# brain-research/l2hmc

Measured on AMD Instinct MI355X. Metric: chain_leapfrog_steps_per_sec, higher is better.
Workload: dtype f32

## Files before the change

### include/l2hmc.h

```cpp
#ifndef L2HMC_H_
#define L2HMC_H_

#include <stdint.h>

#ifdef __cplusplus
extern "C" {
#endif

#define L2HMC_ABI_VERSION 6

enum {
  L2HMC_OK = 0,
  L2HMC_ERR_ARG = -1,
  L2HMC_ERR_UNSUPPORTED = -2,
  L2HMC_ERR_HIP = -3
};

enum {
  L2HMC_ENERGY_GAUSS_DIAG = 1,
  L2HMC_ENERGY_GAUSS_DENSE = 2,
  L2HMC_ENERGY_GMM = 3,
  L2HMC_ENERGY_ROUGHWELL = 4,
  L2HMC_ENERGY_FUNNEL = 5,
  L2HMC_ENERGY_LOGISTIC = 7
// ... 182 lines not shown
  int64_t n_chains;
  int32_t d, H, T;
  const float* x;
  const float* v;
  const uint8_t* direction;
  int32_t direction_all;
  float scale;
  float inv_n;
  float* Lx;
  float* p;
  float* v1;
  float* grad;
  float* workspace;
  int32_t variant;
} L2hmcTrainArgs;

int64_t l2hmc_train_workspace_floats(int64_t n_chains, int32_t d, int32_t H, int32_t T);
int64_t l2hmc_train_grad_floats(int32_t d, int32_t H);
int64_t l2hmc_train_fused_lds_bytes(int32_t energy_kind, int32_t n_comp, int32_t d, int32_t H, int32_t T);
int64_t l2hmc_train_logistic_lds_bytes(int32_t n_data, int32_t d, int32_t H, int32_t T);
int l2hmc_train_propose_grad(const L2hmcTrainArgs* args, void* stream);

typedef struct L2hmcTrainStep {
  const float* x_head;
  int64_t n_head;
  const float* u;
  float* x_next;
  float* terms;
  double* loss;
  float* theta;
// ... 90 lines not shown
```

### l2hmc_amd/_ffi.py

```python
import ctypes as C
import os

_HERE = os.path.dirname(os.path.abspath(__file__))
LIB_PATH = os.path.abspath(os.environ["L2HMC_LIB"]) if os.environ.get("L2HMC_LIB") else os.path.join(_HERE, "csrc", "libl2hmc_hip.so")

ENERGY_GAUSS_DIAG, ENERGY_GAUSS_DENSE, ENERGY_GMM, ENERGY_ROUGHWELL, ENERGY_FUNNEL = 1, 2, 3, 4, 5
ENERGY_LOGISTIC = 7

_fp = C.c_void_p

NET_FIELDS = ("W1", "b1", "W2", "b2", "W3", "b3", "W4", "b4",
              "Ws", "bs", "Wt", "bt", "Wq", "bq", "lam_s", "lam_q")


class L2hmcNet(C.Structure):
    _fields_ = [(k, _fp) for k in NET_FIELDS]


class L2hmcEnergy(C.Structure):
    _fields_ = [("kind", C.c_int32), ("n_comp", C.c_int32), ("mu", _fp), ("prec", _fp),
                ("logc", _fp), ("eta", C.c_float), ("easy", C.c_int32),
                ("temperature", C.c_float), ("anneal_beta", C.c_float),
                ("den", C.c_float), ("reserved_", C.c_int32)]

# ... 99 lines not shown
    "l2hmc_pack_gaussian": (C.c_int, [_fp, C.c_int32, _fp, _fp]),
    "l2hmc_packed_logistic_floats": (C.c_int64, [C.c_int32, C.c_int32]),
    "l2hmc_pack_logistic": (C.c_int, [_fp, _fp, C.c_int32, C.c_int32, _fp, _fp]),
    "l2hmc_trajectory": (C.c_int, [C.POINTER(L2hmcTrajectoryArgs), _fp]),
    "l2hmc_trajectory_ladder": (C.c_int, [C.POINTER(L2hmcTrajectoryArgs), C.POINTER(L2hmcLadderArgs), _fp]),
    "l2hmc_energy": (C.c_int, [C.POINTER(L2hmcEnergy), _fp, C.c_int64, C.c_int32, _fp, _fp, _fp]),
    "l2hmc_p_accept": (C.c_int, [C.POINTER(L2hmcEnergy), _fp, _fp, _fp, _fp, _fp, C.c_int64,
                                 C.c_int32, _fp, _fp]),
    "l2hmc_mh_select": (C.c_int, [_fp, _fp, _fp, _fp, C.c_int64, C.c_int32, _fp, _fp]),
    "l2hmc_loss_terms": (C.c_int, [_fp, C.c_int64, C.c_float, C.c_double, _fp, _fp]),
    "l2hmc_split_workspace_floats": (C.c_int64, [C.c_int64, C.c_int32, C.c_int32, C.c_int32,
                                                 C.POINTER(L2hmcMlp3), C.POINTER(L2hmcMlp3)]),
    "l2hmc_trajectory_split": (C.c_int, [C.POINTER(L2hmcSplitArgs), _fp]),
    "l2hmc_vae_energy": (C.c_int, [C.POINTER(L2hmcMlp3), _fp, _fp, C.c_int64, C.c_int32, _fp, _fp, _fp, C.c_float, _fp]),
    "l2hmc_p_accept_energies": (C.c_int, [_fp, _fp, _fp, _fp, _fp, C.c_int64, C.c_int32, _fp, _fp]),
    "l2hmc_train_workspace_floats": (C.c_int64, [C.c_int64, C.c_int32, C.c_int32, C.c_int32]),
    "l2hmc_train_grad_floats": (C.c_int64, [C.c_int32, C.c_int32]),
    "l2hmc_train_fused_lds_bytes": (C.c_int64, [C.c_int32, C.c_int32, C.c_int32, C.c_int32, C.c_int32]),
    "l2hmc_train_logistic_lds_bytes": (C.c_int64, [C.c_int32, C.c_int32, C.c_int32, C.c_int32]),
    "l2hmc_train_propose_grad": (C.c_int, [C.POINTER(L2hmcTrainArgs), _fp]),
    "l2hmc_train_step": (C.c_int, [C.POINTER(L2hmcTrainArgs), C.POINTER(L2hmcTrainStep), _fp]),
    "l2hmc_adam_step_terms": (C.c_int, [_fp, _fp, _fp, _fp, C.c_int64, C.c_float, C.c_float, C.c_float, C.c_float,
                                        C.c_int64, C.c_int32, _fp, C.c_float, _fp, _fp]),
    "l2hmc_train_split_grad_floats": (C.c_int64, [C.c_int32, C.c_int32, C.POINTER(L2hmcMlp3)]),
    "l2hmc_train_split_workspace_floats": (C.c_int64, [C.c_int64, C.c_int32, C.c_int32, C.c_int32,
                                                       C.POINTER(L2hmcMlp3), C.POINTER(L2hmcMlp3)]),
    "l2hmc_train_split_grad": (C.c_int, [C.POINTER(L2hmcTrainSplitArgs), _fp]),
    "l2hmc_adam_step": (C.c_int, [_fp, _fp, _fp, _fp, C.c_int64, C.c_float, C.c_float, C.c_float, C.c_float,
                                  C.c_int64, C.c_int32, _fp]),
    "l2hmc_ais_begin_step": (C.c_int, [_fp, _fp, _fp, C.c_float, C.c_float, _fp, _fp, C.c_int64, C.c_int32, _fp]),
# ... 68 lines not shown
```

### l2hmc_amd/csrc/l2hmc_abi.hip

```cpp
#include <cstdlib>
#include "traj_tile.hpp"
#include "traj_lane.hpp"

namespace l2hmc {

thread_local char g_err[512] = "";
thread_local char g_kernel[96] = "";
void note_kernel(const char* fmt, long long a, long long b, long long c, long long d) { snprintf(g_kernel, sizeof(g_kernel), fmt, a, b, c, d); }

int fail(int code, const char* fmt, const char* a, long long b, long long c) {
  snprintf(g_err, sizeof(g_err), fmt, a, b, c);
  return code;
}

__global__ void pack_net_kernel(L2hmcNet net, int d, int H, int KH, int NT, float* out) {
  const int idx = blockIdx.x * blockDim.x + threadIdx.x;
  const int ngf = net_groups(NT) * 256;
  if (idx >= net_floats(NT)) return;
  float val = 0.f;
  if (idx < ngf) {
    const int g = idx >> 8, lane = (idx >> 2) & 63, r = idx & 3;
    const int i = lane & 15, q = lane >> 4;
    const int ui = ((i & 3) < KH) ? (i >> 2) * KH + (i & 3) : -1;
    const int uk = (r < KH) ? q * KH + r : -1;
// ... 319 lines not shown
  const int NT = k.NT, DP = 16 * NT, NTp = NW * DT;
  long long o = 0;
  k.o_fw = (int)o;
  o += 2LL * fast_fw_net(NTp, f16);
  k.o_fc = (int)o;
  o += 2LL * fast_fc_net(NTp);
  k.o_rec = (int)o;
  o += 2LL * fast_rec_dir(NTp, k.T);
  k.o_P = (int)o;
  if (NW > 1) o += 2LL * NW * 256;
  k.xb_stride = DP + 4;
  k.o_XB = (int)o;
  if (NW > 1 && (k.ekind == L2HMC_ENERGY_GAUSS_DENSE || k.ekind == L2HMC_ENERGY_GMM)) o += 16LL * k.xb_stride;
  k.o_red = (int)o;
  o += (long long)NW * 16 * 8;
  const int nc = k.ekind == L2HMC_ENERGY_GMM ? k.ncomp : 1;
  k.o_mu = (int)o;
  o += (long long)nc * DP;
  k.o_prec = (int)o;
  if (k.ekind == L2HMC_ENERGY_GAUSS_DIAG) o += DP;
  if (k.ekind == L2HMC_ENERGY_GAUSS_DENSE || k.ekind == L2HMC_ENERGY_GMM) o += (long long)nc * gauss_floats(NT);
  k.o_logc = (int)o;
  o += round4(nc);
  return o * 4;
}

long long plan_lds_tile(KArgs& k, int DT) {
  long long o = 0;
  k.o_fw = (int)o;
  o += 2LL * tile_fw_net(DT);
// ... 297 lines not shown
const char* l2hmc_last_error(void) { return g_err; }

int64_t l2hmc_struct_bytes(int32_t which) {
  switch (which) {
    case L2HMC_STRUCT_NET: return sizeof(L2hmcNet);
    case L2HMC_STRUCT_ENERGY: return sizeof(L2hmcEnergy);
    case L2HMC_STRUCT_TRAJECTORY_ARGS: return sizeof(L2hmcTrajectoryArgs);
    case L2HMC_STRUCT_MLP3: return sizeof(L2hmcMlp3);
    case L2HMC_STRUCT_SPLIT_ARGS: return sizeof(L2hmcSplitArgs);
    case L2HMC_STRUCT_TRAIN_ARGS: return sizeof(L2hmcTrainArgs);
    case L2HMC_STRUCT_TRAIN_SPLIT_ARGS: return sizeof(L2hmcTrainSplitArgs);
    case L2HMC_STRUCT_TRAIN_STEP: return sizeof(L2hmcTrainStep);
    case L2HMC_STRUCT_LADDER_ARGS: return sizeof(L2hmcLadderArgs);
  }
  return fail(L2HMC_ERR_ARG, "l2hmc_struct_bytes: unknown struct id%s");
}

int64_t l2hmc_packed_nets_floats(int32_t d, int32_t H) {
  if (d < 1 || H < 1) return fail(L2HMC_ERR_ARG, "d and H must be >= 1%s");
  if (H > 15) return fail(L2HMC_ERR_UNSUPPORTED, "fused nets support H <= 15 (got %s%lld)", "", H);
  if (d > 512) return fail(L2HMC_ERR_UNSUPPORTED, "fused nets support d <= 512 (got %s%lld)", "", d);
  return 2LL * net_floats(tiles_of(d)) + 2LL * lane_layout(d, H).total + 2LL * net_f16_floats(tiles_of(d));
}

int l2hmc_pack_nets(const L2hmcNet* xnet, const L2hmcNet* vnet, int32_t d, int32_t H,
                    float* packed, void* stream) {
  const int64_t n = l2hmc_packed_nets_floats(d, H);
  if (n < 0) return (int)n;
  if (!xnet || !vnet || !packed) return fail(L2HMC_ERR_ARG, "l2hmc_pack_nets: NULL argument%s");
  const L2hmcNet* nets[2] = {xnet, vnet};
// ... 357 lines not shown
```

### l2hmc_amd/csrc/l2hmc_kernels.hpp

```cpp
#pragma once
#include <hip/hip_runtime.h>
#include <stdint.h>
#include <stdio.h>
#include <string.h>
#include <type_traits>

#include "../../include/l2hmc.h"

namespace l2hmc {

typedef float f4 __attribute__((ext_vector_type(4)));

#define MFMA16(a, b, c) __builtin_amdgcn_mfma_f32_16x16x4f32((a), (b), (c), 0, 0, 0)

__host__ __device__ constexpr bool weights_in_global(int DT) { return DT >= 4; }

int fail(int code, const char* fmt, const char* a = "", long long b = 0, long long c = 0);
inline float roughwell_den(const L2hmcEnergy* e) {
  if (e->den > 0.f) return e->den;
  return e->easy ? e->eta : (float)((double)e->eta * (double)e->eta);
}
void note_kernel(const char* fmt, long long a = 0, long long b = 0, long long c = 0, long long d = 0);
inline bool adam_args_ok(float lr, float beta1, float beta2, float epsilon, int64_t step) {
  return step >= 1 && lr >= 0.f && (beta1 >= 0.f && beta1 < 1.f) && (beta2 >= 0.f && beta2 < 1.f) && epsilon > 0.f;
// ... 50 lines not shown
  long long chain_off;
  int ekind, ncomp, easy;
  const float *mu, *prec, *logc;
  float eta, temperature;
  float den;
  float beta;
  const float *x1, *v1, *logjac_in;
  float *U_out, *grad_out;
  int o_mask, o_trig, o_tb, o_P, o_XB, o_red, o_mu, o_prec, o_logc, xb_stride;
  int o_state;
  const float* ais_beta;
  const float* ais_v0;
  float ais_dbeta, ais_refresh;
  float *ais_w, *ais_alpha;
  int o_fw, o_fc, o_rec;
  unsigned long long* dbg;
};

struct LadArgs {
  int K, M;
  int o_lad;
  float temp[16];
  unsigned long long round0;
  signed char *rung, *trip, *rung_hist;
  const float* u;
  float* cold;
  long long *acc, *att, *trips;
};

#ifdef L2HMC_PHASE_TIMING
// ... 109 lines not shown
  return (fabsf(p) <= 3.402823466e38f) ? p : 0.f;
}

struct U4 { unsigned x, y, z, w; };
__host__ __device__ inline U4 philox4x32_10(U4 c, unsigned k0, unsigned k1) {
#pragma unroll
  for (int i = 0; i < 10; ++i) {
    const unsigned long long p0 = 0xD2511F53ull * c.x, p1 = 0xCD9E8D57ull * c.z;
    const U4 n = {(unsigned)(p1 >> 32) ^ c.y ^ k0, (unsigned)p1, (unsigned)(p0 >> 32) ^ c.w ^ k1, (unsigned)p0};
    c = n;
    k0 += 0x9E3779B9u;
    k1 += 0xBB67AE85u;
  }
  return c;
}
__device__ __forceinline__ f4 philox_normal4(unsigned long long seed, long long gchain, unsigned blk,
                                             unsigned long long prop) {
  const U4 r = philox4x32_10(U4{(unsigned)gchain, blk, (unsigned)prop, (unsigned)(prop >> 32) << 1},
                             (unsigned)seed, (unsigned)(seed >> 32));
  const float k = 5.9604644775390625e-08f;
  const float u1 = ((r.x >> 8) + 1) * k, u2 = (r.y >> 8) * k, u3 = ((r.z >> 8) + 1) * k, u4 = (r.w >> 8) * k;
#ifdef L2HMC_LIBM_NORMALS
  const float ra = sqrtf(-2.f * logf(u1)), rb = sqrtf(-2.f * logf(u3));
  float sa, ca, sb, cb;
  sincosf(6.283185307179586f * u2, &sa, &ca);
  sincosf(6.283185307179586f * u4, &sb, &cb);
#else
  const float m2ln2 = -1.3862943611198906f;
  const float ra = __builtin_amdgcn_sqrtf(m2ln2 * __builtin_amdgcn_logf(u1)), rb = __builtin_amdgcn_sqrtf(m2ln2 * __builtin_amdgcn_logf(u3));
  const float sa = __builtin_amdgcn_sinf(u2), ca = __builtin_amdgcn_cosf(u2), sb = __builtin_amdgcn_sinf(u4), cb = __builtin_amdgcn_cosf(u4);
#endif
  return f4{ra * ca, ra * sa, rb * cb, rb * sb};
}
__device__ __forceinline__ void philox_dir_u(unsigned long long seed, long long gchain,
                                             unsigned long long prop, bool& fwd, float& u) {
  const U4 r = philox4x32_10(U4{(unsigned)gchain, 0u, (unsigned)prop, ((unsigned)(prop >> 32) << 1) | 1u},
                             (unsigned)seed, (unsigned)(seed >> 32));
  fwd = (r.x & 1u) != 0;
  u = (r.y >> 8) * 5.9604644775390625e-08f;
}
__device__ __forceinline__ float philox_swap_u(unsigned long long seed, long long gladder, unsigned long long round, int k) {
  const U4 r = philox4x32_10(U4{(unsigned)gladder, 0xFFFFFFFFu, (unsigned)round,
                                ((unsigned)(round >> 32) << 4) | ((unsigned)(k >> 1) << 1) | 1u},
                             (unsigned)seed, (unsigned)(seed >> 32));
  return (r.x >> 8) * 5.9604644775390625e-08f;
}
template <int DT, int NW>
__device__ __forceinline__ void rng_state(const KArgs& A, long long gchain, unsigned long long prop,
                                          int w, int q, f4 (&z)[DT]) {
#pragma unroll
  for (int t = 0; t < DT; ++t) {
    const int dim0 = 16 * (w * DT + t) + 4 * q;
// ... 368 lines not shown
      const f4 W = Wres[t];
#pragma unroll
      for (int r = 0; r < 4; ++r) acc = MFMA16(W[r], z[t][r], acc);
    } else {
      if (16 * tg < A.d) {
        const f4 W = lds4(wn + ((grp0 + tg) * 64 + lane) * 4);
#pragma unroll
        for (int r = 0; r < 4; ++r)
          acc = MFMA16(W[r], z[t][r], acc);
      }
    }
  }
  return acc;
}

template <int NW, int NP>
__device__ __forceinline__ void xchg(f4 (&p)[NP], const KArgs& A, float* smem, int w, int lane,
                                     int& pb) {
#ifdef L2HMC_ABL_NOXCHG
  return;
#endif
  if (NW > 1) {
    float* P = smem + A.o_P + pb * (NW * NP * 256);
#pragma unroll
    for (int i = 0; i < NP; ++i) *reinterpret_cast<f4*>(P + ((w * NP + i) * 64 + lane) * 4) = p[i];
    __syncthreads();
    f4 part[NP][NW];
#pragma unroll
    for (int i = 0; i < NP; ++i)
#pragma unroll
      for (int ww = 0; ww < NW; ++ww) part[i][ww] = lds4(P + ((ww * NP + i) * 64 + lane) * 4);
    __builtin_amdgcn_sched_barrier(0);
#pragma unroll
    for (int i = 0; i < NP; ++i) {
      f4 sum = part[i][0];
#pragma unroll
      for (int ww = 1; ww < NW; ++ww) sum += part[i][ww];
      p[i] = sum;
    }
    pb ^= 1;
  }
}

template <int DT>
struct TailW {
  static constexpr int NH = DT <= 2 ? DT : 1;
  f4 w2;
// ... 327 lines not shown
```

### l2hmc_amd/csrc/traj_fast.hpp

```cpp
#pragma once
#include "l2hmc_kernels.hpp"
#include "bf3k.hpp"


namespace l2hmc {

__device__ __forceinline__ float relu_i(float a) { return __int_as_float(max(__float_as_int(a), 0)); }
__device__ __forceinline__ f4 rcp4(f4 a) {
  return f4{__builtin_amdgcn_rcpf(a.x), __builtin_amdgcn_rcpf(a.y), __builtin_amdgcn_rcpf(a.z),
            __builtin_amdgcn_rcpf(a.w)};
}
__device__ __forceinline__ f4 ex2_4(f4 a) {
  return f4{__builtin_amdgcn_exp2f(a.x), __builtin_amdgcn_exp2f(a.y), __builtin_amdgcn_exp2f(a.z),
            __builtin_amdgcn_exp2f(a.w)};
}

typedef _Float16 h2v __attribute__((ext_vector_type(2)));
typedef _Float16 h8v __attribute__((ext_vector_type(8)));
typedef float f2v __attribute__((ext_vector_type(2)));
#define L2HMC_F16_SCALE 64.0f
struct WF16 {
  h8v a1;
  h8v a2;
};
__device__ __forceinline__ h2v cvt_pk16(float a, float b) { return __builtin_convertvector(f2v{a, b}, h2v); }
__device__ __forceinline__ h2v lo_pair16(h2v h, float a0, float a1) {
  h2v r;
  const float ns = -L2HMC_F16_SCALE;
  asm("v_fma_mixlo_f16 %0, %1, %2, %3 op_sel:[0,0,0] op_sel_hi:[1,0,0]" : "=v"(r) : "v"(h), "s"(ns), "v"(a0));
  asm("v_fma_mixhi_f16 %0, %1, %2, %3 op_sel:[1,0,0] op_sel_hi:[1,0,0]" : "+v"(r) : "v"(h), "s"(ns), "v"(a1));
  return r;
}
template <bool LAT>
__device__ __forceinline__ h8v split16(f4 a) {
  const f4 ad = a * (1.f / L2HMC_F16_SCALE);
  const h2v h01 = cvt_pk16(ad.x, ad.y), h23 = cvt_pk16(ad.z, ad.w);
  h2v l01, l23;
  if constexpr (LAT) {
    float r0, r1, r2, r3;
    const float ns = -L2HMC_F16_SCALE;
    asm("v_fma_mix_f32 %0, %1, %2, %3 op_sel:[0,0,0] op_sel_hi:[1,0,0]" : "=v"(r0) : "v"(h01), "s"(ns), "v"(a.x));
    asm("v_fma_mix_f32 %0, %1, %2, %3 op_sel:[1,0,0] op_sel_hi:[1,0,0]" : "=v"(r1) : "v"(h01), "s"(ns), "v"(a.y));
    asm("v_fma_mix_f32 %0, %1, %2, %3 op_sel:[0,0,0] op_sel_hi:[1,0,0]" : "=v"(r2) : "v"(h23), "s"(ns), "v"(a.z));
    asm("v_fma_mix_f32 %0, %1, %2, %3 op_sel:[1,0,0] op_sel_hi:[1,0,0]" : "=v"(r3) : "v"(h23), "s"(ns), "v"(a.w));
    l01 = cvt_pk16(r0, r1);
    l23 = cvt_pk16(r2, r3);
  } else {
    l01 = lo_pair16(h01, a.x, a.y);
    l23 = lo_pair16(h23, a.z, a.w);
  }
  return h8v{h01.x, h01.y, h23.x, h23.y, l01.x, l01.y, l23.x, l23.y};
}
__device__ __forceinline__ WF16 wsplit16(f4 w) {
  const float sc = L2HMC_F16_SCALE;
  const h2v h01 = cvt_pk16(w.x, w.y), h23 = cvt_pk16(w.z, w.w);
  const f4 r = f4{w.x - (float)h01.x, w.y - (float)h01.y, w.z - (float)h23.x, w.w - (float)h23.y} * sc;
  const h2v L01 = cvt_pk16(r.x, r.y), L23 = cvt_pk16(r.z, r.w);
  const h2v H01 = cvt_pk16((float)h01.x * sc, (float)h01.y * sc), H23 = cvt_pk16((float)h23.x * sc, (float)h23.y * sc);
  const h2v l01 = cvt_pk16((float)L01.x / sc, (float)L01.y / sc), l23 = cvt_pk16((float)L23.x / sc, (float)L23.y / sc);
// ... 4 lines not shown
}
#define L2HMC_F16_STATE_MAX 2.5e5f
__device__ __forceinline__ float amax4(f4 a) { return fmaxf(fmaxf(fabsf(a.x), fabsf(a.y)), fmaxf(fabsf(a.z), fabsf(a.w))); }
__device__ __forceinline__ f4 mfma16x2(const WF16& W, h8v b, f4 acc) {
  acc = __builtin_amdgcn_mfma_f32_16x16x32_f16(W.a1, b, acc, 0, 0, 0);
  return __builtin_amdgcn_mfma_f32_16x16x32_f16(W.a2, b, acc, 0, 0, 0);
}

__host__ __device__ constexpr int fast_fw_net_f32(int NTp) { return (3 * NTp + 1) * 256; }
__host__ __device__ constexpr int fast_fw_net(int NTp, bool f16 = false) { return (3 * NTp + 1) * (f16 ? 512 : 256); }
__host__ __device__ inline int fast_dpp(int NTp) { return 16 * NTp + 16; }
__host__ __device__ inline int fast_fc_net(int NTp) { return 4 * fast_dpp(NTp); }
__host__ __device__ inline int fast_rec(int NTp) { return 32 + 16 * NTp; }
__host__ __device__ inline int fast_rec_dir(int NTp, int T) { return (T + 2) * fast_rec(NTp) + 16; }

long long plan_lds_fast(KArgs& k, int NW, int DT, bool f16 = false);

#ifndef L2HMC_FAST_SPLIT_LAT_TAIL
#define L2HMC_FAST_SPLIT_LAT_TAIL true
#endif
#ifndef L2HMC_FAST_SPLIT_LAT_PAIR
#define L2HMC_FAST_SPLIT_LAT_PAIR true
#endif
#ifndef L2HMC_FAST_SPLIT_LAT_L1
#define L2HMC_FAST_SPLIT_LAT_L1 false
#endif
template <int DT, bool F16 = false>
struct TailK {
  f4 w2;
  f4 hs[DT], ht[DT], hq[DT];
  f4 cS[DT], cQ[DT], bQ[DT];
};
template <int DT>
struct TailK<DT, true> {
  WF16 w2;
  WF16 hs[DT], ht[DT], hq[DT];
  f4 cS[DT], cQ[DT], bQ[DT];
// ... 26 lines not shown
                                           int w, int lane) {
  const int q = lane >> 4, DPp = fast_dpp(NTp);
  tk.w2 = lds_wf16(fw, NTp, 0, lane);
#pragma unroll
  for (int t = 0; t < DT; ++t) {
    const int tg = w * DT + t;
    tk.hs[t] = lds_wf16(fw, NTp, 1 + 3 * tg + 0, lane);
    tk.ht[t] = lds_wf16(fw, NTp, 1 + 3 * tg + 1, lane);
    tk.hq[t] = lds_wf16(fw, NTp, 1 + 3 * tg + 2, lane);
    tk.cS[t] = lds4(fc + dofs + 16 * tg + 4 * q);
    tk.cQ[t] = lds4(fc + 2 * DPp + 16 * tg + 4 * q);
    tk.bQ[t] = lds4(fc + 3 * DPp + 16 * tg + 4 * q);
  }
}

template <int DT, int KH, class F>
__device__ __forceinline__ void tail_fast(const TailK<DT, false>& tk, f4 hs_, F&& apply) {
  f4 h = splat(0.f);
#pragma unroll
  for (int r = 0; r < KH; ++r) h[r] = relu_i(hs_[r]);
  {
    f4 acc = splat(0.f);
#pragma unroll
    for (int r = 0; r < KH; ++r) acc = MFMA16(tk.w2[r], h[r], acc);
#pragma unroll
    for (int r = 0; r < KH; ++r) h[r] = relu_i(acc[r]);
  }
#pragma unroll
  for (int t = 0; t < DT; ++t) {
    f4 zs = splat(0.f), zt = splat(0.f), zq = splat(0.f);
// ... 7 lines not shown
    __builtin_amdgcn_sched_barrier(0);
#endif
    const f4 rS = rcp4(-(ex2_4(zs) * 0.5f + 0.5f));
    const f4 aS = rS * tk.cS[t] + tk.cS[t];
    const f4 rQ = rcp4(-(ex2_4(zq) * 0.5f + 0.5f));
    const f4 EQ = ex2_4(rQ * tk.cQ[t] + tk.bQ[t]);
    apply(t, aS, zt, EQ);
  }
}
template <int DT, int KH, class F>
__device__ __forceinline__ void tail_fast(const TailK<DT, true>& tk, f4 hs_, F&& apply) {
  f4 h = splat(0.f);
#pragma unroll
  for (int r = 0; r < KH; ++r) h[r] = relu_i(hs_[r]);
  {
    const f4 acc = mfma16x2(tk.w2, split16<L2HMC_FAST_SPLIT_LAT_TAIL>(h), splat(0.f));
#pragma unroll
    for (int r = 0; r < KH; ++r) h[r] = relu_i(acc[r]);
  }
  const h8v b = split16<L2HMC_FAST_SPLIT_LAT_TAIL>(h);
#pragma unroll
  for (int t = 0; t < DT; ++t) {
    f4 zs = __builtin_amdgcn_mfma_f32_16x16x32_f16(tk.hs[t].a1, b, splat(0.f), 0, 0, 0);
    f4 zq = __builtin_amdgcn_mfma_f32_16x16x32_f16(tk.hq[t].a1, b, splat(0.f), 0, 0, 0);
    f4 zt = __builtin_amdgcn_mfma_f32_16x16x32_f16(tk.ht[t].a1, b, splat(0.f), 0, 0, 0);
    zs = __builtin_amdgcn_mfma_f32_16x16x32_f16(tk.hs[t].a2, b, zs, 0, 0, 0);
    zq = __builtin_amdgcn_mfma_f32_16x16x32_f16(tk.hq[t].a2, b, zq, 0, 0, 0);
    zt = __builtin_amdgcn_mfma_f32_16x16x32_f16(tk.ht[t].a2, b, zt, 0, 0, 0);
    const f4 rS = rcp4(-(ex2_4(zs) * 0.5f + 0.5f));
    const f4 aS = rS * tk.cS[t] + tk.cS[t];
    const f4 rQ = rcp4(-(ex2_4(zq) * 0.5f + 0.5f));
    const f4 EQ = ex2_4(rQ * tk.cQ[t] + tk.bQ[t]);
    apply(t, aS, zt, EQ);
  }
}

template <int DT, int KH, class FA, class FB>
__device__ __forceinline__ void tail_fast2(const TailK<DT, true>& tk, f4 hsa, f4 hsb, FA&& applyA, FB&& keepB) {
  f4 ha = splat(0.f), hb = splat(0.f);
#pragma unroll
  for (int r = 0; r < KH; ++r) { ha[r] = relu_i(hsa[r]); hb[r] = relu_i(hsb[r]); }
  {
    const h8v sa = split16<L2HMC_FAST_SPLIT_LAT_PAIR>(ha), sb = split16<L2HMC_FAST_SPLIT_LAT_PAIR>(hb);
    f4 acca = __builtin_amdgcn_mfma_f32_16x16x32_f16(tk.w2.a1, sa, splat(0.f), 0, 0, 0);
    f4 accb = __builtin_amdgcn_mfma_f32_16x16x32_f16(tk.w2.a1, sb, splat(0.f), 0, 0, 0);
    acca = __builtin_amdgcn_mfma_f32_16x16x32_f16(tk.w2.a2, sa, acca, 0, 0, 0);
    accb = __builtin_amdgcn_mfma_f32_16x16x32_f16(tk.w2.a2, sb, accb, 0, 0, 0);
#pragma unroll
    for (int r = 0; r < KH; ++r) { ha[r] = relu_i(acca[r]); hb[r] = relu_i(accb[r]); }
  }
  const h8v ba = split16<L2HMC_FAST_SPLIT_LAT_PAIR>(ha), bb = split16<L2HMC_FAST_SPLIT_LAT_PAIR>(hb);
#pragma unroll
  for (int t = 0; t < DT; ++t) {
    f4 zsa = __builtin_amdgcn_mfma_f32_16x16x32_f16(tk.hs[t].a1, ba, splat(0.f), 0, 0, 0);
    f4 zqa = __builtin_amdgcn_mfma_f32_16x16x32_f16(tk.hq[t].a1, ba, splat(0.f), 0, 0, 0);
    f4 zta = __builtin_amdgcn_mfma_f32_16x16x32_f16(tk.ht[t].a1, ba, splat(0.f), 0, 0, 0);
    f4 zsb = __builtin_amdgcn_mfma_f32_16x16x32_f16(tk.hs[t].a1, bb, splat(0.f), 0, 0, 0);
    f4 zqb = __builtin_amdgcn_mfma_f32_16x16x32_f16(tk.hq[t].a1, bb, splat(0.f), 0, 0, 0);
    f4 ztb = __builtin_amdgcn_mfma_f32_16x16x32_f16(tk.ht[t].a1, bb, splat(0.f), 0, 0, 0);
    zsa = __builtin_amdgcn_mfma_f32_16x16x32_f16(tk.hs[t].a2, ba, zsa, 0, 0, 0);
    zqa = __builtin_amdgcn_mfma_f32_16x16x32_f16(tk.hq[t].a2, ba, zqa, 0, 0, 0);
    zta = __builtin_amdgcn_mfma_f32_16x16x32_f16(tk.ht[t].a2, ba, zta, 0, 0, 0);
    zsb = __builtin_amdgcn_mfma_f32_16x16x32_f16(tk.hs[t].a2, bb, zsb, 0, 0, 0);
    zqb = __builtin_amdgcn_mfma_f32_16x16x32_f16(tk.hq[t].a2, bb, zqb, 0, 0, 0);
    ztb = __builtin_amdgcn_mfma_f32_16x16x32_f16(tk.ht[t].a2, bb, ztb, 0, 0, 0);
    const f4 rSa = rcp4(-(ex2_4(zsa) * 0.5f + 0.5f));
// ... 177 lines not shown
    }
  }
  PT_DECL;
  PT_MARK(0);
  pv[0] = vnet_l1(x, g);
  xchg<NW, 1>(pv, A, smem, w, lane, pb);

  const long long gchain = A.chain_off + chain;
  const bool rng_v = (A.rng_flags & L2HMC_RNG_V) != 0, rng_d = (A.rng_flags & L2HMC_RNG_DIR) != 0;
  const bool rng_u = (A.rng_flags & L2HMC_RNG_U) != 0;
  f4 vn[DT];
  if (!rng_v) load_state<DT, NW>(A.v, A, chain, live, w, q, vn);
  bool fwd_n = (A.dir != nullptr && !rng_d) ? (live ? A.dir[chain] != 0 : true) : (A.dir_all != 0);
  float u_n = (A.u != nullptr && !rng_u && live) ? A.u[chain] : 0.f;
  const bool have_u = A.u != nullptr || rng_u;
  for (int m = 0; m < A.M; ++m) {
    const long long moff = (long long)m * A.N;
    const unsigned long long prop = A.rng_prop0 + (unsigned long long)m;
    if (rng_v) {
      rng_state<DT, NW>(A, gchain, prop, w, q, v);
    } else {
#pragma unroll
      for (int t = 0; t < DT; ++t) v[t] = vn[t];
    }
    bool fwd = fwd_n;
    float u_m = u_n;
    if (rng_d || rng_u) {
      bool fr;
      float ur;
      philox_dir_u(A.rng_seed, gchain, prop, fr, ur);
      if (rng_d) fwd = fr;
      if (rng_u) u_m = ur;
    }
    if (m + 1 < A.M) {
      if (!rng_v) load_state<DT, NW>(A.v + (moff + A.N) * A.d, A, chain, live, w, q, vn);
      if (A.dir != nullptr && !rng_d && live) fwd_n = A.dir[moff + A.N + chain] != 0;
      if (A.u != nullptr && !rng_u && live) u_n = A.u[moff + A.N + chain];
    }
    constexpr bool KEEP_G0 = EK != L2HMC_ENERGY_GAUSS_DIAG;
    f4 x0[DT], g0[KEEP_G0 ? DT : 1];
#pragma unroll
    for (int t = 0; t < DT; ++t) {
      x0[t] = x[t];
      if constexpr (KEEP_G0) g0[t] = g[t];
    }
    const f4 pv0 = pv[0];
    float red[F16 ? 6 : 5];
    float amax_l = 0.f;
    if constexpr (F16) {
#pragma unroll
      for (int t = 0; t < DT; ++t) amax_l = fmaxf(amax_l, fmaxf(amax4(x[t]), fmaxf(amax4(v[t]), amax4(g[t]))));
    }
    red[0] = U_start;
    red[1] = 0.f;
#pragma unroll
    for (int t = 0; t < DT; ++t) red[1] += 0.5f * hsum(v[t] * v[t]);
    red[2] = 0.f;
    f4 ldv = splat(0.f);

    const float ff = fwd ? 1.f : 0.f, nf = ff - 1.f;
    const int dofs = fwd ? 0 : DPp;
    const int row0 = fwd ? A.step_begin : (A.T - 1 - A.step_begin);
    const float* rec = smem + A.o_rec + (fwd ? RECD : 0) + (row0 + 1) * R + 4 * q;
    const int drec = fwd ? R : -R;
    f4 tbv = lds4(rec + 16);

    constexpr bool RT = DT == 1 || PK == 1;
    TailK<DT, F16> tkx;
    if constexpr (RT) load_tailk<DT>(tkx, fwx, fcx, dofs, NTp, w, lane);
    const TailK<DT, F16>& TKX = *(RT ? &tkx : &tk);
    load_tailk<DT>(tk, fwv, fcv, dofs, NTp, w, lane);
#ifndef L2HMC_FAST_SERIAL_TAILS
#ifndef L2HMC_FAST_PAIR_DT2
#define L2HMC_FAST_PAIR_DT2 0
#endif
    constexpr bool PAIR = F16 && RT && (DT == 1 || L2HMC_FAST_PAIR_DT2);
#else
    constexpr bool PAIR = false;
#endif
    f4 aS_n[DT], T_n[DT], EQ_n[DT];
    if constexpr (PAIR) {
      tail_fast<DT, KH>(tk, pv[0] + tbv, [&](int t, f4 aS, f4 T, f4 EQ) { aS_n[t] = aS; T_n[t] = T; EQ_n[t] = EQ; });
    }
    for (int it = 0; it < A.n_steps; ++it) {
      f4 k1[DT], vh[DT], y[DT], xin[DT];
      const f4 tbx = lds4(rec);
// ... 17 lines not shown
      }
      PT_MARK(2);

      if constexpr (!RT) load_tailk<DT>(tk, fwx, fcx, dofs, NTp, w, lane);
#pragma unroll
      for (int t = 0; t < DT; ++t) xin[t] = k1[t] * x[t];
      f4 pa, px[1];
      if constexpr (F16) {
        pa = l1_part16<DT>(vh, Z, l1h.xa);
        px[0] = l1_part16<DT>(xin, pa, l1h.xb);
      } else {
        pa = l1_part<DT, NW>(nullptr, 0, A, w, lane, vh, Z, l1w.xa);
        px[0] = pa + l1_part<DT, NW>(nullptr, NT, A, w, lane, xin, Z, l1w.xb);
      }
      PT_MARK(3);
      xchg<NW, 1>(px, A, smem, w, lane, pb);
      PT_MARK(4);
      tail_fast<DT, KH>(TKX, px[0] + tbx, [&](int t, f4 aS, f4 T, f4 EQ) {
        const f4 up = 1.f - k1[t];
        const f4 aSm = up * aS;
        const f4 ES = ex2_4(aSm);
        ldv += aSm;
        const f4 tr = up * (EQ * vh[t] + T);
        y[t] = ES * (nf * tr + x[t]) + ff * tr;
        xin[t] = up * y[t];
      });
      PT_MARK(5);
      f4 py[1];
      if constexpr (F16) py[0] = l1_part16<DT>(xin, pa, l1h.xb);
      else py[0] = pa + l1_part<DT, NW>(nullptr, NT, A, w, lane, xin, Z, l1w.xb);
      PT_MARK(6);
      xchg<NW, 1>(py, A, smem, w, lane, pb);
      PT_MARK(7);
      tail_fast<DT, KH>(TKX, py[0] + tbx, [&](int t, f4 aS, f4 T, f4 EQ) {
        const f4 aSm = k1[t] * aS;
        const f4 ES = ex2_4(aSm);
        ldv += aSm;
        const f4 tr = k1[t] * (EQ * vh[t] + T);
        x[t] = ES * (nf * tr + y[t]) + ff * tr;
      });
      PT_MARK(8);

      if constexpr (!RT) load_tailk<DT>(tk, fwv, fcv, dofs, NTp, w, lane);
      grad(x, g, red[2], need_p && it == A.n_steps - 1);
      pv[0] = vnet_l1(x, g);
      PT_MARK(9);
      xchg<NW, 1>(pv, A, smem, w, lane, pb);
      PT_MARK(10);
      auto vhalf2 = [&](int t, f4 aS, f4 T, f4 EQ) {
        const f4 ES = ex2_4(aS);
        ldv += aS;
        const f4 tr = T - EQ * g[t];
        v[t] = ES * (nf * tr + vh[t]) + ff * tr;
      };
      if constexpr (PAIR) {
        tail_fast2<DT, KH>(tk, pv[0] + tbv, pv[0] + tbv_n, vhalf2, [&](int t, f4 aS, f4 T, f4 EQ) { aS_n[t] = aS; T_n[t] = T; EQ_n[t] = EQ; });
      } else {
        tail_fast<DT, KH>(tk, pv[0] + tbv, vhalf2);
      }
      PT_MARK(11);
      tbv = tbv_n;
    }
    if constexpr (EK == L2HMC_ENERGY_GAUSS_DIAG) red[2] = diag_U(x, g);
    const float ld = hsum(ldv) * 0.6931471805599453f;

    const bool last = m == A.M - 1;
    red[3] = 0.f;
#pragma unroll
    for (int t = 0; t < DT; ++t) red[3] += 0.5f * hsum(v[t] * v[t]);
    red[4] = ld;
    const float U_end = red[2];
    if constexpr (F16) {
#pragma unroll
      for (int t = 0; t < DT; ++t) amax_l = fmaxf(amax_l, fmaxf(amax4(x[t]), fmaxf(amax4(v[t]), amax4(g[t]))));
      red[5] = amax_l < L2HMC_F16_STATE_MAX ? 0.f : 1.f;
    }
    chain_allreduce<NW, F16 ? 6 : 5>(red, smem + A.o_red, w, lane);
    if constexpr (F16) {
      if (red[5] > 0.f) {
        const float qnan = __uint_as_float(0x7fc00000u);
#pragma unroll
        for (int t = 0; t < DT; ++t) { x[t] = splat(qnan); v[t] = splat(qnan); }
        red[4] = qnan;
      }
    }
    if (last) {
      store_state<DT, NW>(A.x_out, A, chain, live, w, q, x);
      store_state<DT, NW>(A.v_out, A, chain, live, w, q, v);
    }
    const bool writer = live && w == 0 && lane < 16;
    if (A.logjac_out != nullptr && writer) A.logjac_out[moff + chain] = red[4];
// ... 28 lines not shown
```

Measured before the change: 2.350 billion.

## Interleave next-proposal Philox rounds into exchange waits and keep tail weights resident

Result: slower. 2.299 billion (-2.2%).

```diff
diff --git a/include/l2hmc.h b/include/l2hmc.h
--- a/include/l2hmc.h
+++ b/include/l2hmc.h
@@ -220,6 +220,9 @@
   float* workspace;
   int32_t variant;
 } L2hmcTrainArgs;
+
+int64_t l2hmc_traj_fast_lds_bytes(int32_t energy_kind, int32_t d, int32_t T, int32_t n_waves, int32_t tiles_per_wave,
+                                  int32_t f16x2);
 
 int64_t l2hmc_train_workspace_floats(int64_t n_chains, int32_t d, int32_t H, int32_t T);
 int64_t l2hmc_train_grad_floats(int32_t d, int32_t H);
diff --git a/l2hmc_amd/_ffi.py b/l2hmc_amd/_ffi.py
--- a/l2hmc_amd/_ffi.py
+++ b/l2hmc_amd/_ffi.py
@@ -137,6 +137,7 @@
     "l2hmc_trajectory_split": (C.c_int, [C.POINTER(L2hmcSplitArgs), _fp]),
     "l2hmc_vae_energy": (C.c_int, [C.POINTER(L2hmcMlp3), _fp, _fp, C.c_int64, C.c_int32, _fp, _fp, _fp, C.c_float, _fp]),
     "l2hmc_p_accept_energies": (C.c_int, [_fp, _fp, _fp, _fp, _fp, C.c_int64, C.c_int32, _fp, _fp]),
+    "l2hmc_traj_fast_lds_bytes": (C.c_int64, [C.c_int32, C.c_int32, C.c_int32, C.c_int32, C.c_int32, C.c_int32]),
     "l2hmc_train_workspace_floats": (C.c_int64, [C.c_int64, C.c_int32, C.c_int32, C.c_int32]),
     "l2hmc_train_grad_floats": (C.c_int64, [C.c_int32, C.c_int32]),
     "l2hmc_train_fused_lds_bytes": (C.c_int64, [C.c_int32, C.c_int32, C.c_int32, C.c_int32, C.c_int32]),
diff --git a/l2hmc_amd/csrc/l2hmc_abi.hip b/l2hmc_amd/csrc/l2hmc_abi.hip
--- a/l2hmc_amd/csrc/l2hmc_abi.hip
+++ b/l2hmc_amd/csrc/l2hmc_abi.hip
@@ -357,6 +357,8 @@
   if (NW > 1 && (k.ekind == L2HMC_ENERGY_GAUSS_DENSE || k.ekind == L2HMC_ENERGY_GMM)) o += 16LL * k.xb_stride;
   k.o_red = (int)o;
   o += (long long)NW * 16 * 8;
+  k.o_park = (int)o;
+  o += fast_park_floats(k.ekind, NW, DT, f16);
   const int nc = k.ekind == L2HMC_ENERGY_GMM ? k.ncomp : 1;
   k.o_mu = (int)o;
   o += (long long)nc * DP;
@@ -684,6 +686,18 @@
     case L2HMC_STRUCT_LADDER_ARGS: return sizeof(L2hmcLadderArgs);
   }
   return fail(L2HMC_ERR_ARG, "l2hmc_struct_bytes: unknown struct id%s");
+}
+
+int64_t l2hmc_traj_fast_lds_bytes(int32_t ek, int32_t d, int32_t T, int32_t n_waves, int32_t tiles_per_wave, int32_t f16x2) {
+  if (d < 1 || T < 1 || n_waves < 1 || tiles_per_wave < 1 || tiles_per_wave > 2 || n_waves * tiles_per_wave < tiles_of(d))
+    return fail(L2HMC_ERR_ARG, "l2hmc_traj_fast_lds_bytes: bad argument (d, T >= 1; 1 or 2 tiles per wave; waves x tiles >= ceil(d / 16))%s");
+  KArgs k{};
+  k.d = d;
+  k.T = T;
+  k.NT = tiles_of(d);
+  k.ekind = ek;
+  k.ncomp = 1;
+  return plan_lds_fast(k, n_waves, tiles_per_wave, f16x2 != 0);
 }
 
 int64_t l2hmc_packed_nets_floats(int32_t d, int32_t H) {
diff --git a/l2hmc_amd/csrc/l2hmc_kernels.hpp b/l2hmc_amd/csrc/l2hmc_kernels.hpp
--- a/l2hmc_amd/csrc/l2hmc_kernels.hpp
+++ b/l2hmc_amd/csrc/l2hmc_kernels.hpp
@@ -88,6 +88,7 @@
   float ais_dbeta, ais_refresh;
   float *ais_w, *ais_alpha;
   int o_fw, o_fc, o_rec;
+  int o_park;
   unsigned long long* dbg;
 };
 
@@ -227,10 +228,19 @@
   }
   return c;
 }
-__device__ __forceinline__ f4 philox_normal4(unsigned long long seed, long long gchain, unsigned blk,
-                                             unsigned long long prop) {
-  const U4 r = philox4x32_10(U4{(unsigned)gchain, blk, (unsigned)prop, (unsigned)(prop >> 32) << 1},
-                             (unsigned)seed, (unsigned)(seed >> 32));
+__device__ __forceinline__ void philox_round(U4& c, unsigned long long seed, int i) {
+  const unsigned k0 = (unsigned)seed + (unsigned)i * 0x9E3779B9u, k1 = (unsigned)(seed >> 32) + (unsigned)i * 0xBB67AE85u;
+  const unsigned long long p0 = 0xD2511F53ull * c.x, p1 = 0xCD9E8D57ull * c.z;
+  const U4 n = {(unsigned)(p1 >> 32) ^ c.y ^ k0, (unsigned)p1, (unsigned)(p0 >> 32) ^ c.w ^ k1, (unsigned)p0};
+  c = n;
+}
+__device__ __forceinline__ U4 philox_ctr_normal(long long gchain, unsigned blk, unsigned long long prop) {
+  return U4{(unsigned)gchain, blk, (unsigned)prop, (unsigned)(prop >> 32) << 1};
+}
+__device__ __forceinline__ U4 philox_ctr_dir_u(long long gchain, unsigned long long prop) {
+  return U4{(unsigned)gchain, 0u, (unsigned)prop, ((unsigned)(prop >> 32) << 1) | 1u};
+}
+__device__ __forceinline__ f4 philox_normal4_of(U4 r) {
   const float k = 5.9604644775390625e-08f;
   const float u1 = ((r.x >> 8) + 1) * k, u2 = (r.y >> 8) * k, u3 = ((r.z >> 8) + 1) * k, u4 = (r.w >> 8) * k;
 #ifdef L2HMC_LIBM_NORMALS
@@ -245,10 +255,13 @@
 #endif
   return f4{ra * ca, ra * sa, rb * cb, rb * sb};
 }
+__device__ __forceinline__ f4 philox_normal4(unsigned long long seed, long long gchain, unsigned blk,
+                                             unsigned long long prop) {
+  return philox_normal4_of(philox4x32_10(philox_ctr_normal(gchain, blk, prop), (unsigned)seed, (unsigned)(seed >> 32)));
+}
 __device__ __forceinline__ void philox_dir_u(unsigned long long seed, long long gchain,
                                              unsigned long long prop, bool& fwd, float& u) {
-  const U4 r = philox4x32_10(U4{(unsigned)gchain, 0u, (unsigned)prop, ((unsigned)(prop >> 32) << 1) | 1u},
-                             (unsigned)seed, (unsigned)(seed >> 32));
+  const U4 r = philox4x32_10(philox_ctr_dir_u(gchain, prop), (unsigned)seed, (unsigned)(seed >> 32));
   fwd = (r.x & 1u) != 0;
   u = (r.y >> 8) * 5.9604644775390625e-08f;
 }
@@ -647,9 +660,12 @@
   return acc;
 }
 
-template <int NW, int NP>
+struct XchgNoHook {
+  __device__ __forceinline__ void operator()() const {}
+};
+template <int NW, int NP, class HOOK = XchgNoHook>
 __device__ __forceinline__ void xchg(f4 (&p)[NP], const KArgs& A, float* smem, int w, int lane,
-                                     int& pb) {
+                                     int& pb, HOOK&& hook = HOOK{}) {
 #ifdef L2HMC_ABL_NOXCHG
   return;
 #endif
@@ -664,6 +680,10 @@
 #pragma unroll
       for (int ww = 0; ww < NW; ++ww) part[i][ww] = lds4(P + ((ww * NP + i) * 64 + lane) * 4);
     __builtin_amdgcn_sched_barrier(0);
+    if constexpr (!std::is_same_v<std::decay_t<HOOK>, XchgNoHook>) {
+      hook();
+      __builtin_amdgcn_sched_barrier(0);
+    }
 #pragma unroll
     for (int i = 0; i < NP; ++i) {
       f4 sum = part[i][0];
diff --git a/l2hmc_amd/csrc/traj_fast.hpp b/l2hmc_amd/csrc/traj_fast.hpp
--- a/l2hmc_amd/csrc/traj_fast.hpp
+++ b/l2hmc_amd/csrc/traj_fast.hpp
@@ -31,7 +31,7 @@
   asm("v_fma_mixhi_f16 %0, %1, %2, %3 op_sel:[1,0,0] op_sel_hi:[1,0,0]" : "+v"(r) : "v"(h), "s"(ns), "v"(a1));
   return r;
 }
-template <bool LAT>
+template <bool LAT, int KH = 4>
 __device__ __forceinline__ h8v split16(f4 a) {
   const f4 ad = a * (1.f / L2HMC_F16_SCALE);
   const h2v h01 = cvt_pk16(ad.x, ad.y), h23 = cvt_pk16(ad.z, ad.w);
@@ -42,7 +42,8 @@
     asm("v_fma_mix_f32 %0, %1, %2, %3 op_sel:[0,0,0] op_sel_hi:[1,0,0]" : "=v"(r0) : "v"(h01), "s"(ns), "v"(a.x));
     asm("v_fma_mix_f32 %0, %1, %2, %3 op_sel:[1,0,0] op_sel_hi:[1,0,0]" : "=v"(r1) : "v"(h01), "s"(ns), "v"(a.y));
     asm("v_fma_mix_f32 %0, %1, %2, %3 op_sel:[0,0,0] op_sel_hi:[1,0,0]" : "=v"(r2) : "v"(h23), "s"(ns), "v"(a.z));
-    asm("v_fma_mix_f32 %0, %1, %2, %3 op_sel:[1,0,0] op_sel_hi:[1,0,0]" : "=v"(r3) : "v"(h23), "s"(ns), "v"(a.w));
+    if constexpr (KH <= 3) r3 = 0.f;
+    else asm("v_fma_mix_f32 %0, %1, %2, %3 op_sel:[1,0,0] op_sel_hi:[1,0,0]" : "=v"(r3) : "v"(h23), "s"(ns), "v"(a.w));
     l01 = cvt_pk16(r0, r1);
     l23 = cvt_pk16(r2, r3);
   } else {
@@ -77,6 +78,18 @@
 __host__ __device__ inline int fast_rec(int NTp) { return 32 + 16 * NTp; }
 __host__ __device__ inline int fast_rec_dir(int NTp, int T) { return (T + 2) * fast_rec(NTp) + 16; }
 
+
+#ifndef L2HMC_FAST_RESIDENT_LAUNCH
+#define L2HMC_FAST_RESIDENT_LAUNCH 1
+#endif
+#ifndef L2HMC_FAST_RNG_AHEAD
+#define L2HMC_FAST_RNG_AHEAD 1
+#endif
+__host__ __device__ constexpr bool fast_rng_ahead(int ek, int NW, int DT, bool f16) {
+  return L2HMC_FAST_RNG_AHEAD && ek == L2HMC_ENERGY_GAUSS_DIAG && f16 && DT == 1 && NW > 1;
+}
+__host__ __device__ constexpr int fast_park_floats(int ek, int NW, int DT, bool f16) { return fast_rng_ahead(ek, NW, DT, f16) ? (NW + 1) * 256 : 0; }
+
 long long plan_lds_fast(KArgs& k, int NW, int DT, bool f16 = false);
 
 #ifndef L2HMC_FAST_SPLIT_LAT_TAIL
@@ -84,6 +97,9 @@
 #endif
 #ifndef L2HMC_FAST_SPLIT_LAT_PAIR
 #define L2HMC_FAST_SPLIT_LAT_PAIR true
+#endif
+#ifndef L2HMC_FAST_SPLIT_KH
+#define L2HMC_FAST_SPLIT_KH 1
 #endif
 #ifndef L2HMC_FAST_SPLIT_LAT_L1
 #define L2HMC_FAST_SPLIT_LAT_L1 false
@@ -140,6 +156,13 @@
   }
 }
 
+template <int DT, bool F16>
+__device__ __forceinline__ void load_tailk_dir(TailK<DT, F16>& tk, const float* fc, int dofs, int w, int lane) {
+  const int q = lane >> 4;
+#pragma unroll
+  for (int t = 0; t < DT; ++t) tk.cS[t] = lds4(fc + dofs + 16 * (w * DT + t) + 4 * q);
+}
+
 template <int DT, int KH, class F>
 __device__ __forceinline__ void tail_fast(const TailK<DT, false>& tk, f4 hs_, F&& apply) {
   f4 h = splat(0.f);
@@ -177,11 +200,11 @@
 #pragma unroll
   for (int r = 0; r < KH; ++r) h[r] = relu_i(hs_[r]);
   {
-    const f4 acc = mfma16x2(tk.w2, split16<L2HMC_FAST_SPLIT_LAT_TAIL>(h), splat(0.f));
+    const f4 acc = mfma16x2(tk.w2, split16<L2HMC_FAST_SPLIT_LAT_TAIL, L2HMC_FAST_SPLIT_KH ? KH : 4>(h), splat(0.f));
 #pragma unroll
     for (int r = 0; r < KH; ++r) h[r] = relu_i(acc[r]);
   }
-  const h8v b = split16<L2HMC_FAST_SPLIT_LAT_TAIL>(h);
+  const h8v b = split16<L2HMC_FAST_SPLIT_LAT_TAIL, L2HMC_FAST_SPLIT_KH ? KH : 4>(h);
 #pragma unroll
   for (int t = 0; t < DT; ++t) {
     f4 zs = __builtin_amdgcn_mfma_f32_16x16x32_f16(tk.hs[t].a1, b, splat(0.f), 0, 0, 0);
@@ -204,7 +227,7 @@
 #pragma unroll
   for (int r = 0; r < KH; ++r) { ha[r] = relu_i(hsa[r]); hb[r] = relu_i(hsb[r]); }
   {
-    const h8v sa = split16<L2HMC_FAST_SPLIT_LAT_PAIR>(ha), sb = split16<L2HMC_FAST_SPLIT_LAT_PAIR>(hb);
+    const h8v sa = split16<L2HMC_FAST_SPLIT_LAT_PAIR, L2HMC_FAST_SPLIT_KH ? KH : 4>(ha), sb = split16<L2HMC_FAST_SPLIT_LAT_PAIR, L2HMC_FAST_SPLIT_KH ? KH : 4>(hb);
     f4 acca = __builtin_amdgcn_mfma_f32_16x16x32_f16(tk.w2.a1, sa, splat(0.f), 0, 0, 0);
     f4 accb = __builtin_amdgcn_mfma_f32_16x16x32_f16(tk.w2.a1, sb, splat(0.f), 0, 0, 0);
     acca = __builtin_amdgcn_mfma_f32_16x16x32_f16(tk.w2.a2, sa, acca, 0, 0, 0);
@@ -212,7 +235,7 @@
 #pragma unroll
     for (int r = 0; r < KH; ++r) { ha[r] = relu_i(acca[r]); hb[r] = relu_i(accb[r]); }
   }
-  const h8v ba = split16<L2HMC_FAST_SPLIT_LAT_PAIR>(ha), bb = split16<L2HMC_FAST_SPLIT_LAT_PAIR>(hb);
+  const h8v ba = split16<L2HMC_FAST_SPLIT_LAT_PAIR, L2HMC_FAST_SPLIT_KH ? KH : 4>(ha), bb = split16<L2HMC_FAST_SPLIT_LAT_PAIR, L2HMC_FAST_SPLIT_KH ? KH : 4>(hb);
 #pragma unroll
   for (int t = 0; t < DT; ++t) {
     f4 zsa = __builtin_amdgcn_mfma_f32_16x16x32_f16(tk.hs[t].a1, ba, splat(0.f), 0, 0, 0);
@@ -420,23 +443,77 @@
   bool fwd_n = (A.dir != nullptr && !rng_d) ? (live ? A.dir[chain] != 0 : true) : (A.dir_all != 0);
   float u_n = (A.u != nullptr && !rng_u && live) ? A.u[chain] : 0.f;
   const bool have_u = A.u != nullptr || rng_u;
+  constexpr bool RT = DT == 1 || PK == 1;
+  constexpr bool RL = RT && L2HMC_FAST_RESIDENT_LAUNCH;
+  TailK<DT, F16> tkx;
+  if constexpr (RL) {
+    load_tailk<DT>(tkx, fwx, fcx, 0, NTp, w, lane);
+    load_tailk<DT>(tk, fwv, fcv, 0, NTp, w, lane);
+  }
+  constexpr bool AHEAD = fast_rng_ahead(EK, NW, DT, F16);
+  U4 cc = {0u, 0u, 0u, 0u}, rn = {0u, 0u, 0u, 0u};
+  const int tick_end = (rng_d || rng_u) ? 20 : 10;
+  int tick = tick_end;
+  unsigned long long prop_a = 0ull;
+  auto ahead_begin = [&](unsigned long long prop) {
+    prop_a = prop;
+    tick = rng_v ? 0 : 10;
+    cc = rng_v ? philox_ctr_normal(gchain, (unsigned)(4 * w + q), prop)
+               : philox_ctr_dir_u(gchain, prop);
+  };
+  auto ahead_round = [&]() {
+    if (tick < tick_end) {
+      philox_round(cc, A.rng_seed, tick < 10 ? tick : tick - 10);
+      ++tick;
+      if (tick == 10) {
+        __builtin_amdgcn_sched_barrier(0);
+        rn = cc;
+        cc = philox_ctr_dir_u(gchain, prop_a);
+      }
+    }
+  };
+  auto ahead_end = [&](f4& vv, bool& fr, float& ur) {
+    while (tick < tick_end) ahead_round();
+    if (rng_v) {
+      const int dim0 = 16 * w + 4 * q;
+      const f4 n = philox_normal4_of(rn);
+      vv = f4{dim0 + 0 < A.d ? n.x : 0.f, dim0 + 1 < A.d ? n.y : 0.f, dim0 + 2 < A.d ? n.z : 0.f, dim0 + 3 < A.d ? n.w : 0.f};
+    }
+    fr = (cc.x & 1u) != 0;
+    ur = (cc.y >> 8) * 5.9604644775390625e-08f;
+  };
+  const bool rng_any = rng_v || rng_d || rng_u;
+  bool fr_n = false;
+  float ur_n = 0.f;
   for (int m = 0; m < A.M; ++m) {
     const long long moff = (long long)m * A.N;
     const unsigned long long prop = A.rng_prop0 + (unsigned long long)m;
-    if (rng_v) {
-      rng_state<DT, NW>(A, gchain, prop, w, q, v);
-    } else {
-#pragma unroll
-      for (int t = 0; t < DT; ++t) v[t] = vn[t];
-    }
     bool fwd = fwd_n;
     float u_m = u_n;
-    if (rng_d || rng_u) {
-      bool fr;
-      float ur;
-      philox_dir_u(A.rng_seed, gchain, prop, fr, ur);
-      if (rng_d) fwd = fr;
-      if (rng_u) u_m = ur;
+    if constexpr (AHEAD) {
+      if (m == 0 && rng_any) {
+        ahead_begin(prop);
+        ahead_end(vn[0], fr_n, ur_n);
+      }
+#pragma unroll
+      for (int t = 0; t < DT; ++t) v[t] = vn[t];
+      if (rng_d) fwd = fr_n;
+      if (rng_u) u_m = ur_n;
+      if (rng_any && m + 1 < A.M) ahead_begin(prop + 1ull);
+    } else {
+      if (rng_v) {
+        rng_state<DT, NW>(A, gchain, prop, w, q, v);
+      } else {
+#pragma unroll
+        for (int t = 0; t < DT; ++t) v[t] = vn[t];
+      }
+      if (rng_d || rng_u) {
+        bool fr;
+        float ur;
+        philox_dir_u(A.rng_seed, gchain, prop, fr, ur);
+        if (rng_d) fwd = fr;
+        if (rng_u) u_m = ur;
+      }
     }
     if (m + 1 < A.M) {
       if (!rng_v) load_state<DT, NW>(A.v + (moff + A.N) * A.d, A, chain, live, w, q, vn);
@@ -445,12 +522,19 @@
     }
     constexpr bool KEEP_G0 = EK != L2HMC_ENERGY_GAUSS_DIAG;
     f4 x0[DT], g0[KEEP_G0 ? DT : 1];
+    f4 pv0;
+    if constexpr (!AHEAD) pv0 = pv[0];
+    float* const park_x = smem + A.o_park + tid * 4;
+    float* const park_pv = smem + A.o_park + NW * 256 + lane * 4;
 #pragma unroll
     for (int t = 0; t < DT; ++t) {
-      x0[t] = x[t];
+      if constexpr (!AHEAD) x0[t] = x[t];
       if constexpr (KEEP_G0) g0[t] = g[t];
     }
-    const f4 pv0 = pv[0];
+    if constexpr (AHEAD) {
+      *reinterpret_cast<f4*>(park_x) = x[0];
+      *reinterpret_cast<f4*>(park_pv) = pv[0];
+    }
     float red[F16 ? 6 : 5];
     float amax_l = 0.f;
     if constexpr (F16) {
@@ -471,11 +555,18 @@
     const int drec = fwd ? R : -R;
     f4 tbv = lds4(rec + 16);
 
-    constexpr bool RT = DT == 1 || PK == 1;
-    TailK<DT, F16> tkx;
-    if constexpr (RT) load_tailk<DT>(tkx, fwx, fcx, dofs, NTp, w, lane);
+    if constexpr (RL) {
+      load_tailk_dir<DT, F16>(tkx, fcx, dofs, w, lane);
+      load_tailk_dir<DT, F16>(tk, fcv, dofs, w, lane);
+    } else {
+      if constexpr (RT) load_tailk<DT>(tkx, fwx, fcx, dofs, NTp, w, lane);
+      load_tailk<DT>(tk, fwv, fcv, dofs, NTp, w, lane);
+    }
     const TailK<DT, F16>& TKX = *(RT ? &tkx : &tk);
-    load_tailk<DT>(tk, fwv, fcv, dofs, NTp, w, lane);
+    auto xch = [&](f4 (&pp)[1]) {
+      if constexpr (AHEAD) xchg<NW, 1>(pp, A, smem, w, lane, pb, ahead_round);
+      else xchg<NW, 1>(pp, A, smem, w, lane, pb);
+    };
 #ifndef L2HMC_FAST_SERIAL_TAILS
 #ifndef L2HMC_FAST_PAIR_DT2
 #define L2HMC_FAST_PAIR_DT2 0
@@ -523,7 +614,7 @@
         px[0] = pa + l1_part<DT, NW>(nullptr, NT, A, w, lane, xin, Z, l1w.xb);
       }
       PT_MARK(3);
-      xchg<NW, 1>(px, A, smem, w, lane, pb);
+      xch(px);
       PT_MARK(4);
       tail_fast<DT, KH>(TKX, px[0] + tbx, [&](int t, f4 aS, f4 T, f4 EQ) {
         const f4 up = 1.f - k1[t];
@@ -539,7 +630,7 @@
       if constexpr (F16) py[0] = l1_part16<DT>(xin, pa, l1h.xb);
       else py[0] = pa + l1_part<DT, NW>(nullptr, NT, A, w, lane, xin, Z, l1w.xb);
       PT_MARK(6);
-      xchg<NW, 1>(py, A, smem, w, lane, pb);
+      xch(py);
       PT_MARK(7);
       tail_fast<DT, KH>(TKX, py[0] + tbx, [&](int t, f4 aS, f4 T, f4 EQ) {
         const f4 aSm = k1[t] * aS;
@@ -554,7 +645,7 @@
       grad(x, g, red[2], need_p && it == A.n_steps - 1);
       pv[0] = vnet_l1(x, g);
       PT_MARK(9);
-      xchg<NW, 1>(pv, A, smem, w, lane, pb);
+      xch(pv);
       PT_MARK(10);
       auto vhalf2 = [&](int t, f4 aS, f4 T, f4 EQ) {
         const f4 ES = ex2_4(aS);
@@ -584,6 +675,11 @@
       for (int t = 0; t < DT; ++t) amax_l = fmaxf(amax_l, fmaxf(amax4(x[t]), fmaxf(amax4(v[t]), amax4(g[t]))));
       red[5] = amax_l < L2HMC_F16_STATE_MAX ? 0.f : 1.f;
     }
+    if constexpr (AHEAD) {
+      x0[0] = lds4(park_x);
+      pv0 = lds4(park_pv);
+      if (rng_any && !last) ahead_end(vn[0], fr_n, ur_n);
+    }
     chain_allreduce<NW, F16 ? 6 : 5>(red, smem + A.o_red, w, lane);
     if constexpr (F16) {
       if (red[5] > 0.f) {
```
